# samxuxiang/BrepGen

Measured on NVIDIA H100. Metric: B-reps/sec (1000-step ABC cascade), higher is better.
Workload: dtype f16 x f16 -> f32 (wgmma; split hi+lo weights on in/out-proj; fp32 residual/LN/softmax)

## Files before the change

### brepgen_b200/_ffi.py

```python
from __future__ import annotations

import ctypes as C
import os
from typing import Optional

_HERE = os.path.dirname(os.path.abspath(__file__))
LIB_PATH = os.environ.get("BG_LIB", os.path.join(_HERE, "libbrepgen_b200.so"))

vp, i32, i64, u64, f32, sz = C.c_void_p, C.c_int, C.c_int64, C.c_uint64, C.c_float, C.c_size_t


class BgNamedTensor(C.Structure):
    _fields_ = [("name", C.c_char_p), ("data", vp), ("numel", i64)]


class BgDenoiserArgs(C.Structure):
    _fields_ = [("B", i32), ("S", i32), ("E", i32), ("x", vp), ("timesteps", vp), ("n_timesteps", i32),
                ("surfPos", vp), ("surfZ", vp), ("edgePos", vp), ("mask", vp), ("class_label", vp), ("out", vp), ("compact", i32)]


SIGNATURES = {
    "bg_version": (i32, []),
    "bg_last_error": (C.c_char_p, []),
    "bg_check_device": (i32, []),
    "bg_launch_count": (u64, []),
    "bg_denoiser_create": (i32, [i32, i32, i32, C.POINTER(BgNamedTensor), i32, vp, vp, C.POINTER(vp)]),
    "bg_denoiser_destroy": (None, [vp]),
    "bg_denoiser_workspace_bytes": (sz, [vp, i32, i32, i32]),
    "bg_denoiser_forward": (i32, [vp, C.POINTER(BgDenoiserArgs), vp, sz, vp]),
    "bg_vae_create": (i32, [i32, C.POINTER(BgNamedTensor), i32, vp, C.POINTER(vp)]),
    "bg_vae_destroy": (None, [vp]),
    "bg_vae_workspace_bytes": (sz, [vp, i32]),
    "bg_vae_decode": (i32, [vp, vp, i32, vp, vp, sz, vp]),
    "bg_vae_decode_hw": (i32, [vp, vp, i32, i32, vp, vp, sz, vp]),
    "bg_vae_encode": (i32, [vp, vp, i32, i32, vp, vp, sz, vp]),
    "bg_ddpm_step": (i32, [vp, vp, f32, vp, vp, vp, u64, u64, i64, f32, f32, f32, f32, f32, f32, vp]),
    "bg_ddpm_step_tab": (i32, [vp, vp, f32, vp, vp, u64, u64, u64, i64, vp, vp, f32, vp]),
    "bg_step_advance": (i32, [vp, i32, vp, vp, vp]),
    "bg_pndm_step": (i32, [vp, vp, i64, f32, f32, vp, f32, vp, f32, vp, f32, vp, f32, vp]),
    "bg_axpby": (i32, [vp, f32, vp, f32, vp, i64, vp]),
    "bg_dedup_surfaces": (i32, [vp, i32, i32, f32, vp, vp, vp]),
    "bg_dedup_edges": (i32, [vp, vp, i32, i32, i32, f32, vp, vp]),
    "bg_edge_endpoints": (i32, [vp, vp, f32, i64, vp, vp]),
    "bg_nn_exclude": (i32, [vp, vp, vp, i32, vp, vp]),
    "bg_pairs_within": (i32, [vp, i32, f32, vp, vp]),
    "bg_edge_pair_match": (i32, [vp, vp, i32, i32, f32, vp, vp]),
    "bg_edge_fit": (i32, [vp, vp, i32, vp, vp]),
    "bg_surf_init": (i32, [vp, vp, vp, vp, vp, i32, vp, vp]),
    "bg_surf_offset_opt": (i32, [vp, vp, vp, vp, vp, i32, i32, i32, f32, f32, f32, f32, f32, vp, vp, vp]),
    "bg_op_gemm_f16": (i32, [vp, i32, vp, i32, i32, i32, i32, vp, i32, i32, i32, vp, vp, i32, vp, i32, i32, vp]),
    "bg_op_attention": (i32, [vp, vp, i32, i32, vp, i32, vp, vp]),
    "bg_op_layernorm_f16": (i32, [vp, i32, vp, vp, vp, i32, i32, i32, vp]),
    "bg_op_cast_f16": (i32, [vp, vp, i64, vp]),
}

_lib: Optional[C.CDLL] = None


def lib() -> C.CDLL:
    global _lib
    if _lib is None:
        if not os.path.exists(LIB_PATH):
            raise RuntimeError(f"{LIB_PATH} not found: build it with `python -c 'import __graft_entry__ as g; g.build()'` "
                               "(brepgen_b200 has no CPU / PyTorch fallback)")
        l = C.CDLL(LIB_PATH)
        for name, (res, args) in SIGNATURES.items():
            fn = getattr(l, name)
            fn.restype, fn.argtypes = res, args
        _lib = l
    return _lib


def check(status: int, what: str = "") -> None:
    if status != 0:
        msg = lib().bg_last_error().decode(errors="replace")
        raise RuntimeError(f"brepgen_b200 {what} failed (status {status}): {msg}")


def ptr(t) -> Optional[int]:
    return None if t is None else t.data_ptr()


def named_tensors(state_dict, device):
    import torch
    arr = (BgNamedTensor * len(state_dict))()
    for i, (k, v) in enumerate(state_dict.items()):
        if v.device != device or v.dtype != torch.float32 or not v.is_contiguous():
            raise RuntimeError(f"parameter {k} must be contiguous fp32 on {device} (call .to(device) first)")
        arr[i].name, arr[i].data, arr[i].numel = k.encode(), v.data_ptr(), v.numel()
    return arr


def current_stream() -> int:
    import torch
    return torch.cuda.current_stream().cuda_stream


replayed_launches = 0


def note_replay(launches_per_replay: int, times: int = 1) -> None:
    global replayed_launches
    replayed_launches += int(launches_per_replay) * int(times)
```

### brepgen_b200/csrc/api.cu

```cuda
#include "../../include/brepgen_b200.h"
#include "bg_internal.h"

namespace bg {
const char* last_error_cstr();
}
using namespace bg;

extern "C" {

int bg_version(void) { return 100; }

const char* bg_last_error(void) { return last_error_cstr(); }

uint64_t bg_launch_count(void) { return launch_count(); }

int bg_check_device(void) {
  int dev = 0, major = 0, minor = 0;
  BG_CUDA(cudaGetDevice(&dev));
  BG_CUDA(cudaDeviceGetAttribute(&major, cudaDevAttrComputeCapabilityMajor, dev));
  BG_CUDA(cudaDeviceGetAttribute(&minor, cudaDevAttrComputeCapabilityMinor, dev));
  if (major != 9 || minor != 0)
    return set_error(BG_ERR_UNSUPPORTED_ARCH, "brepgen_b200 kernels are built for sm_90a (H100) only; device is sm_" +
                                                  std::to_string(major) + std::to_string(minor));
  return BG_OK;
}

int bg_op_gemm_f16(const void* A, int lda, const void* W, int ldw, int M, int N, int K, void* out, int ldo, int out_f16,
                   int relu, const float* bias, const float* resid, int ldr, const float* rowvec, int rows_per_vec,
                   int ldv, void* stream) {
  BG_TRY(bg_check_device());
  GemmEpilogue ep;
  ep.out = out; ep.ldo = ldo; ep.out_f16 = out_f16; ep.relu = relu; ep.bias = bias;
  ep.resid = resid; ep.ldr = ldr; ep.rowvec = rowvec; ep.rows_per_vec = rows_per_vec; ep.ldv = ldv;
  return launch_gemm_f16(reinterpret_cast<cudaStream_t>(stream), reinterpret_cast<const __half*>(A), lda,
                         reinterpret_cast<const __half*>(W), ldw, M, N, K, ep);
}

int bg_op_attention(const void* qkv, void* out, int B, int L, const uint8_t* key_mask, int use_block_list,
                    int* scratch_int, void* stream) {
  BG_TRY(bg_check_device());
  cudaStream_t st = reinterpret_cast<cudaStream_t>(stream);
  AttnArgs a;
  a.qkv = reinterpret_cast<const __half*>(qkv);
  a.out = reinterpret_cast<__half*>(out);
  a.ldo = 768; a.B = B; a.L = L; a.key_mask = key_mask;
  if (use_block_list && key_mask) {
    BG_REQUIRE(scratch_int != nullptr, "attention: block list needs scratch_int");
    const int nkb = (L + 127) / 128;
    a.blk_list = scratch_int;
    a.blk_count = scratch_int + (size_t)B * nkb;
    uint32_t* words = reinterpret_cast<uint32_t*>(scratch_int + (size_t)B * (nkb + 1));
    a.blk_words = words;
    BG_TRY(launch_build_block_list(st, key_mask, B, L, scratch_int, scratch_int + (size_t)B * nkb, words));
  }
  return launch_attention(st, a);
}

int bg_op_layernorm_f16(const float* x, int ldx, const float* gamma, const float* beta, void* y, int ldy, int rows,
                        int act, void* stream) {
  return launch_layernorm_f16(reinterpret_cast<cudaStream_t>(stream), x, ldx, gamma, beta, reinterpret_cast<__half*>(y),
                              ldy, rows, act);
}

int bg_op_cast_f16(const float* x, void* y, int64_t n, void* stream) {
  return launch_cast_f32_to_f16(reinterpret_cast<cudaStream_t>(stream), x, reinterpret_cast<__half*>(y), (size_t)n);
}

}
```

### brepgen_b200/csrc/attn.cu

```cuda
#include <math.h>

#include "bg_internal.h"
#include "ptx.cuh"


namespace bg {

namespace {

constexpr int DH = 64;
constexpr int NHEAD = 12;
constexpr int DMODEL = 768;
constexpr int BQ = 128;
constexpr int TILE_BYTES = 128 * DH * 2;
constexpr int ST = 2;
constexpr int OFF_Q = 0;
constexpr int OFF_K = TILE_BYTES;
constexpr int OFF_V = OFF_K + ST * TILE_BYTES;
constexpr int OFF_BAR = OFF_V + ST * TILE_BYTES;
constexpr int OFF_MASKW = OFF_BAR + 256;
constexpr int MAX_KB = 64;
constexpr int SMEM_BYTES = OFF_MASKW + MAX_KB * 16 + 1024;
constexpr int THREADS = 384;
constexpr int CONSUMER_THREADS = 256;

struct AttnParams {
  __half* out;
  int ldo;
  int B, L, nkb;
  const uint8_t* key_mask;
  const int* blk_list;
  const int* blk_count;
  const uint32_t* blk_words;
  const int* seq_row0;
  const int* seq_len;
  float scale_log2;
};

__device__ __forceinline__ float quad_max(float v) {
  v = fmaxf(v, __shfl_xor_sync(0xffffffffu, v, 1));
  return fmaxf(v, __shfl_xor_sync(0xffffffffu, v, 2));
}
__device__ __forceinline__ float quad_sum(float v) {
  v += __shfl_xor_sync(0xffffffffu, v, 1);
  return v + __shfl_xor_sync(0xffffffffu, v, 2);
}

__global__ void __launch_bounds__(THREADS, 1)
attn_kernel(const __grid_constant__ CUtensorMap tmQKV, const AttnParams p) {
  extern __shared__ uint8_t smem_raw[];
  uint8_t* smem = reinterpret_cast<uint8_t*>((reinterpret_cast<uintptr_t>(smem_raw) + 1023) & ~uintptr_t(1023));
  uint64_t* bars = reinterpret_cast<uint64_t*>(smem + OFF_BAR);
  uint64_t* q_full = bars;
  uint64_t* k_full = q_full + 1;
  uint64_t* k_empty = k_full + ST;
  uint64_t* v_full = k_empty + ST;
  uint64_t* v_empty = v_full + ST;

  const int warp = threadIdx.x >> 5;
  const int lane = threadIdx.x & 31;
  const int wg = threadIdx.x >> 7;
  const int qgrp = blockIdx.x, h = blockIdx.y, b = blockIdx.z;
  const int row0 = p.seq_row0 ? p.seq_row0[b] : b * p.L;
  const int len = p.seq_len ? p.seq_len[b] : p.L;
  if (qgrp * BQ >= len) return;
  const int nblk = p.blk_count ? p.blk_count[b] : (len + 127) / 128;
  const int* blist = p.blk_list ? p.blk_list + (size_t)b * p.nkb : nullptr;

  if (threadIdx.x == 0) {
    tma_prefetch_desc(&tmQKV);
    mbar_init(q_full, 1);
    for (int i = 0; i < ST; ++i) {
      mbar_init(&k_full[i], 1);
      mbar_init(&k_empty[i], CONSUMER_THREADS);
      mbar_init(&v_full[i], 1);
      mbar_init(&v_empty[i], CONSUMER_THREADS);
    }
    fence_barrier_init();
  }
  uint32_t* maskw = reinterpret_cast<uint32_t*>(smem + OFF_MASKW);
  if (p.blk_words || !p.key_mask) {
    for (int wi = threadIdx.x; wi < nblk * 4; wi += THREADS) {
      uint32_t w;
      if (p.blk_words) {
        w = p.blk_words[((size_t)b * p.nkb + (wi >> 2)) * 4 + (wi & 3)];
      } else {
        const int base = (wi >> 2) * 128 + (wi & 3) * 32;
        w = base + 32 <= len ? 0u : (base >= len ? 0xffffffffu : (0xffffffffu << (len - base)));
      }
      maskw[wi] = w;
    }
  } else {
    for (int wi = warp; wi < nblk * 4; wi += THREADS / 32) {
      const int kb = blist ? blist[wi >> 2] : (wi >> 2);
      const int key = kb * 128 + (wi & 3) * 32 + lane;
      bool bad = key >= len;
      if (!bad) bad = p.key_mask[(size_t)b * p.L + key] != 0;
      const uint32_t w = __ballot_sync(0xffffffffu, bad);
      if (lane == 0) maskw[wi] = w;
    }
  }
  __syncthreads();

  if (wg == 0) {
    setmaxnreg_dec<24>();
    if (warp == 0 && elect_one()) {
      mbar_arrive_expect_tx(q_full, TILE_BYTES);
      tma_load_2d(smem + OFF_Q, &tmQKV, q_full, h * DH, row0 + qgrp * BQ);
      for (int it = 0; it < nblk; ++it) {
        const int kb = blist ? blist[it] : it;
        const int s = it % ST;
        const uint32_t par = ((it / ST) & 1) ^ 1;
        mbar_wait(&k_empty[s], par);
        mbar_arrive_expect_tx(&k_full[s], TILE_BYTES);
        tma_load_2d(smem + OFF_K + s * TILE_BYTES, &tmQKV, &k_full[s], DMODEL + h * DH, row0 + kb * 128);
        mbar_wait(&v_empty[s], par);
        mbar_arrive_expect_tx(&v_full[s], TILE_BYTES);
        tma_load_2d(smem + OFF_V + s * TILE_BYTES, &tmQKV, &v_full[s], 2 * DMODEL + h * DH, row0 + kb * 128);
      }
    }
    return;
  }

  setmaxnreg_inc<240>();
  const int half = wg - 1;
  const int wq = warp & 3;
  const float c = p.scale_log2;
  const uint32_t q_addr = smem_u32(smem + OFF_Q) + half * 64 * 128;
  float m_run[2] = {-INFINITY, -INFINITY}, l_run[2] = {0.f, 0.f};
  float o[DH / 2];
#pragma unroll
  for (int i = 0; i < DH / 2; ++i) o[i] = 0.f;

  mbar_wait(q_full, 0);
  for (int it = 0; it < nblk; ++it) {
    const int s = it % ST;
    const uint32_t par = (it / ST) & 1;
    float sc[64];
    mbar_wait(&k_full[s], par);
    const uint32_t k_addr = smem_u32(smem + OFF_K + s * TILE_BYTES);
    wgmma_fence();
#pragma unroll
    for (int k = 0; k < DH / 16; ++k)
      wgmma_m64n128k16_ss(sc, make_sw128_desc(q_addr + k * 32), make_sw128_desc(k_addr + k * 32), k > 0 ? 1u : 0u);
    wgmma_commit();
    wgmma_wait<0>();
    wgmma_fence_operand(sc);
    mbar_arrive(&k_empty[s]);

    const uint4 iw = *reinterpret_cast<const uint4*>(maskw + it * 4);
    if ((iw.x | iw.y | iw.z | iw.w) != 0) {
      const uint32_t inval[4] = {iw.x, iw.y, iw.z, iw.w};
#pragma unroll
      for (int i = 0; i < 16; ++i)
#pragma unroll
        for (int j = 0; j < 2; ++j) {
          const int key = 8 * i + 2 * (lane & 3) + j;
          if ((inval[key >> 5] >> (key & 31)) & 1u) {
            sc[4 * i + j] = -INFINITY;
            sc[4 * i + 2 + j] = -INFINITY;
          }
        }
    }
    float ref[2], alpha[2];
#pragma unroll
    for (int hr = 0; hr < 2; ++hr) {
      float mx = -INFINITY;
#pragma unroll
      for (int i = 0; i < 16; ++i) mx = fmaxf(mx, fmaxf(sc[4 * i + 2 * hr], sc[4 * i + 2 * hr + 1]));
      const float m_new = fmaxf(m_run[hr], quad_max(mx));
      ref[hr] = m_new == -INFINITY ? 0.f : m_new;
      alpha[hr] = ex2((m_run[hr] - ref[hr]) * c);
      m_run[hr] = m_new;
      l_run[hr] *= alpha[hr];
    }
#pragma unroll
    for (int i = 0; i < DH / 8; ++i) {
      o[4 * i] *= alpha[0];
      o[4 * i + 1] *= alpha[0];
      o[4 * i + 2] *= alpha[1];
      o[4 * i + 3] *= alpha[1];
    }
    uint32_t pa[8][4];
    const float nm0 = -ref[0] * c, nm1 = -ref[1] * c;
#pragma unroll
    for (int i = 0; i < 16; ++i) {
      const float p0 = ex2(fmaf(sc[4 * i], c, nm0)), p1 = ex2(fmaf(sc[4 * i + 1], c, nm0));
      const float p2 = ex2(fmaf(sc[4 * i + 2], c, nm1)), p3 = ex2(fmaf(sc[4 * i + 3], c, nm1));
      l_run[0] += p0 + p1;
      l_run[1] += p2 + p3;
      pa[i >> 1][(i & 1) * 2] = pack_half2(p0, p1);
      pa[i >> 1][(i & 1) * 2 + 1] = pack_half2(p2, p3);
    }

    mbar_wait(&v_full[s], par);
    const uint32_t v_addr = smem_u32(smem + OFF_V + s * TILE_BYTES);
    wgmma_fence_operand(o);
    wgmma_fence();
#pragma unroll
    for (int kk = 0; kk < 8; ++kk) wgmma_m64n64k16_rs_bt(o, pa[kk], make_sw128_desc(v_addr + kk * 2048), 1u);
    wgmma_commit();
    wgmma_wait<0>();
    wgmma_fence_operand(o);
    mbar_arrive(&v_empty[s]);
  }

#pragma unroll
  for (int hr = 0; hr < 2; ++hr) {
    const float l = quad_sum(l_run[hr]);
    const float inv = l > 0.f ? 1.f / l : 0.f;
    const int row = qgrp * BQ + half * 64 + wq * 16 + hr * 8 + (lane >> 2);
    if (row >= len) continue;
    __half* dst = p.out + ((size_t)row0 + row) * p.ldo + h * DH + 2 * (lane & 3);
#pragma unroll
    for (int i = 0; i < DH / 8; ++i)
      *reinterpret_cast<uint32_t*>(dst + 8 * i) = pack_half2(o[4 * i + 2 * hr] * inv, o[4 * i + 2 * hr + 1] * inv);
  }
}

__global__ void block_list_kernel(const uint8_t* __restrict__ key_mask, int L, int nkb, int* __restrict__ blk_list,
                                  int* __restrict__ blk_count, uint32_t* __restrict__ blk_words) {
  extern __shared__ int sm_bl[];
  int* pos = sm_bl;
  uint32_t* wds = reinterpret_cast<uint32_t*>(sm_bl + nkb);
  const int b = blockIdx.x;
  const int warp = threadIdx.x >> 5, lane = threadIdx.x & 31, nwarp = blockDim.x >> 5;
  for (int kb = warp; kb < nkb; kb += nwarp) {
    bool any = false;
#pragma unroll
    for (int c = 0; c < 4; ++c) {
      const int key = kb * 128 + c * 32 + lane;
      const bool bad = key >= L || key_mask[(size_t)b * L + key] != 0;
      const uint32_t w = __ballot_sync(0xffffffffu, bad);
      any = any || w != 0xffffffffu;
      if (lane == 0) wds[kb * 4 + c] = w;
    }
    if (lane == 0) pos[kb] = any ? 0 : -1;
  }
  __syncthreads();
  if (threadIdx.x == 0) {
    int n = 0;
    for (int kb = 0; kb < nkb; ++kb)
      if (pos[kb] == 0) {
        blk_list[(size_t)b * nkb + n] = kb;
        pos[kb] = n++;
      }
    blk_count[b] = n;
  }
  __syncthreads();
  if (blk_words)
    for (int i = threadIdx.x; i < nkb * 4; i += blockDim.x)
      if (pos[i >> 2] >= 0) blk_words[((size_t)b * nkb + pos[i >> 2]) * 4 + (i & 3)] = wds[i];
}

}

int launch_attention(cudaStream_t st, const AttnArgs& a) {
  BG_REQUIRE(a.qkv && a.out && a.B > 0 && a.L > 0, "attention: bad arguments");
  BG_REQUIRE(a.ldo % 8 == 0, "attention: output pitch must be a multiple of 8");
  BG_REQUIRE(a.L <= 128 * MAX_KB, "attention: sequence longer than 8192 tokens is not supported");
  BG_REQUIRE((a.blk_list == nullptr) == (a.blk_count == nullptr), "attention: blk_list and blk_count go together");
  CUtensorMap tm;
  BG_REQUIRE((a.seq_row0 == nullptr) == (a.seq_len == nullptr), "attention: seq_row0 and seq_len go together");
  BG_REQUIRE(a.seq_len == nullptr || (a.key_mask == nullptr && a.blk_list == nullptr), "attention: variable-length mode takes no mask");
  BG_TRY(make_tmap_2d_f16(&tm, a.qkv, (uint64_t)a.B * (uint64_t)a.L, 3 * DMODEL, 3 * DMODEL, 128));
  AttnParams p;
  p.out = a.out; p.ldo = a.ldo; p.B = a.B; p.L = a.L; p.nkb = (a.L + 127) / 128;
  p.key_mask = a.key_mask; p.blk_list = a.blk_list; p.blk_count = a.blk_count; p.blk_words = a.blk_words;
  p.seq_row0 = a.seq_row0; p.seq_len = a.seq_len;
  p.scale_log2 = 1.4426950408889634f / 8.0f;
  BG_TRY(ensure_dynamic_smem(reinterpret_cast<const void*>(&attn_kernel), SMEM_BYTES));
  dim3 grid((a.L + BQ - 1) / BQ, NHEAD, a.B);
  attn_kernel<<<grid, THREADS, SMEM_BYTES, st>>>(tm, p);
  return check_launch("attn_kernel launch");
}

int launch_build_block_list(cudaStream_t st, const uint8_t* key_mask, int B, int L, int* blk_list, int* blk_count,
                            uint32_t* blk_words) {
  BG_REQUIRE(key_mask && blk_list && blk_count && B > 0 && L > 0, "block list: bad arguments");
  const int nkb = (L + 127) / 128;
  block_list_kernel<<<B, 128, nkb * 5 * sizeof(int), st>>>(key_mask, L, nkb, blk_list, blk_count, blk_words);
  return check_launch("block_list_kernel launch");
}

}
```

### include/brepgen_b200.h

```cpp
#ifndef BREPGEN_B200_H_
#define BREPGEN_B200_H_

#include <stddef.h>
#include <stdint.h>

#ifdef __cplusplus
extern "C" {
#endif

typedef enum {
  BG_STATUS_OK = 0,
  BG_STATUS_BAD_ARG = -1,
  BG_STATUS_UNSUPPORTED_ARCH = -2,
  BG_STATUS_CUDA = -3,
  BG_STATUS_WORKSPACE = -4,
  BG_STATUS_MISSING_WEIGHT = -5
} BgStatus;

int bg_version(void);
const char* bg_last_error(void);
uint64_t bg_launch_count(void);
int bg_check_device(void);

typedef struct BgDenoiser BgDenoiser;

typedef struct {
  const char* name;
  const float* data;
  int64_t numel;
} BgNamedTensor;

int bg_denoiser_create(int kind, int use_cf, int precision, const BgNamedTensor* weights, int n_weights,
                       const float* sincos, void* stream, BgDenoiser** out);
void bg_denoiser_destroy(BgDenoiser* m);

typedef struct {
  int B, S, E;
  const float* x;
  const int64_t* timesteps;
  int n_timesteps;
  const float* surfPos;
  const float* surfZ;
  const float* edgePos;
  const uint8_t* mask;
  const int64_t* class_label;
  float* out;
  int compact;
} BgDenoiserArgs;

size_t bg_denoiser_workspace_bytes(const BgDenoiser* m, int B, int S, int E);
int bg_denoiser_forward(BgDenoiser* m, const BgDenoiserArgs* args, void* workspace, size_t workspace_bytes,
                        void* stream);

typedef struct BgVae BgVae;
int bg_vae_create(int kind, const BgNamedTensor* weights, int n_weights, void* stream, BgVae** out);
void bg_vae_destroy(BgVae* m);
size_t bg_vae_workspace_bytes(const BgVae* m, int N);
int bg_vae_decode(BgVae* m, const float* z, int N, float* out, void* workspace, size_t workspace_bytes, void* stream);
int bg_vae_decode_hw(BgVae* m, const float* z, int N, int hw, float* out, void* workspace, size_t workspace_bytes,
                     void* stream);
int bg_vae_encode(BgVae* m, const float* x, int N, int hw, float* out, void* workspace, size_t workspace_bytes,
                  void* stream);

int bg_ddpm_step(const float* eps_cond, const float* eps_uncond, float cfg_w, const float* x, float* out,
                 const float* noise, uint64_t seed, uint64_t offset, int64_t n, float sqrt_one_minus_abar,
                 float sqrt_abar, float clip, float c_x0, float c_x, float sigma, void* stream);
int bg_ddpm_step_tab(const float* eps_cond, const float* eps_uncond, float cfg_w, const float* x, float* out, uint64_t seed,
                     uint64_t offset0, uint64_t offset_stride, int64_t n, const float* coef_table, const int32_t* step,
                     float clip, void* stream);
int bg_step_advance(const int64_t* timesteps, int n_steps, int32_t* step, int64_t* t_cur, void* stream);
int bg_pndm_step(const float* x, float* out, int64_t n, float c_sample, float c_eps, const float* e0, float w0,
                 const float* e1, float w1, const float* e2, float w2, const float* e3, float w3, void* stream);
int bg_axpby(const float* x, float a, const float* y, float b, float* out, int64_t n, void* stream);

int bg_dedup_surfaces(const float* surfPos, int B, int S, float threshold, float* out_pos, uint8_t* out_mask, void* stream);
int bg_dedup_edges(const float* edgePos, const uint8_t* surf_mask, int B, int S, int E, float threshold,
                   uint8_t* edge_mask, void* stream);

int bg_op_gemm_f16(const void* A, int lda, const void* W, int ldw, int M, int N, int K, void* out, int ldo, int out_f16,
                   int relu, const float* bias, const float* resid, int ldr, const float* rowvec, int rows_per_vec,
                   int ldv, void* stream);
int bg_op_attention(const void* qkv, void* out, int B, int L, const uint8_t* key_mask, int use_block_list,
                    int* scratch_int, void* stream);
int bg_op_layernorm_f16(const float* x, int ldx, const float* gamma, const float* beta, void* y, int ldy, int rows,
                        int act, void* stream);
int bg_op_cast_f16(const float* x, void* y, int64_t n, void* stream);

int bg_edge_endpoints(const float* edge_ncs, const float* edge_pos, float pos_scale, int64_t n_edges, float* out, void* stream);
int bg_nn_exclude(const float* pts, const int32_t* group, const int32_t* seg_off, int n_seg, int32_t* nn, void* stream);
int bg_pairs_within(const float* pts, int n, float threshold, uint8_t* out, void* stream);
int bg_edge_pair_match(const int32_t* edge_vertex_adj, const float* z, int z_dim, int n, float threshold, uint8_t* out,
                       void* stream);
int bg_edge_fit(const float* edge_ncs, const float* vertex_se, int n_edges, float* edge_wcs, void* stream);
int bg_surf_init(const float* surf_ncs, const float* surf_pos, const float* edge_wcs, const int32_t* adj_off, const int32_t* adj,
                 int n_faces, float* surf_wcs, void* stream);
int bg_surf_offset_opt(const float* surf_init, const float* edge_wcs, const int32_t* adj_off, const int32_t* adj,
                       const float* inv_nface, int n_faces, int max_edges_per_face, int iters, float lr, float beta1, float beta2,
                       float eps, float weight_decay, float* surf_out, float* offset_out, void* stream);

#ifdef __cplusplus
}
#endif
#endif
```

Measured before the change: 0.1608.

## Software-pipeline attention QK and PV wgmma across key blocks; add varlen entry

Restructures the attention consumer loop so the QK^T wgmma for block it is issued together with the PV wgmma for block it-1, letting softmax of one block overlap tensor-core work of the next. Stage and phase bookkeeping moves into a small ring struct, and the softmax, rescale and pack steps are factored into helpers. It also adds a variable-length attention API that passes per-sequence row offsets and lengths. This adds register pressure (sc, pa and o are live together) and more complex barrier ordering for the V buffers. The varlen path relies on AttnArgs fields and kernel support that are not visible here.

```diff
diff --git a/brepgen_b200/_ffi.py b/brepgen_b200/_ffi.py
--- a/brepgen_b200/_ffi.py
+++ b/brepgen_b200/_ffi.py
@@ -50,6 +50,7 @@
     "bg_surf_offset_opt": (i32, [vp, vp, vp, vp, vp, i32, i32, i32, f32, f32, f32, f32, f32, vp, vp, vp]),
     "bg_op_gemm_f16": (i32, [vp, i32, vp, i32, i32, i32, i32, vp, i32, i32, i32, vp, vp, i32, vp, i32, i32, vp]),
     "bg_op_attention": (i32, [vp, vp, i32, i32, vp, i32, vp, vp]),
+    "bg_op_attention_varlen": (i32, [vp, vp, i32, i32, vp, vp, vp]),
     "bg_op_layernorm_f16": (i32, [vp, i32, vp, vp, vp, i32, i32, i32, vp]),
     "bg_op_cast_f16": (i32, [vp, vp, i64, vp]),
 }
diff --git a/brepgen_b200/csrc/api.cu b/brepgen_b200/csrc/api.cu
--- a/brepgen_b200/csrc/api.cu
+++ b/brepgen_b200/csrc/api.cu
@@ -56,6 +56,18 @@
   return launch_attention(st, a);
 }
 
+int bg_op_attention_varlen(const void* qkv, void* out, int B, int L, const int* seq_row0, const int* seq_len,
+                           void* stream) {
+  BG_TRY(bg_check_device());
+  BG_REQUIRE(seq_row0 && seq_len, "attention: variable-length mode needs seq_row0 and seq_len");
+  AttnArgs a;
+  a.qkv = reinterpret_cast<const __half*>(qkv);
+  a.out = reinterpret_cast<__half*>(out);
+  a.ldo = 768; a.B = B; a.L = L;
+  a.seq_row0 = seq_row0; a.seq_len = seq_len;
+  return launch_attention(reinterpret_cast<cudaStream_t>(stream), a);
+}
+
 int bg_op_layernorm_f16(const float* x, int ldx, const float* gamma, const float* beta, void* y, int ldy, int rows,
                         int act, void* stream) {
   return launch_layernorm_f16(reinterpret_cast<cudaStream_t>(stream), x, ldx, gamma, beta, reinterpret_cast<__half*>(y),
diff --git a/brepgen_b200/csrc/attn.cu b/brepgen_b200/csrc/attn.cu
--- a/brepgen_b200/csrc/attn.cu
+++ b/brepgen_b200/csrc/attn.cu
@@ -46,6 +46,90 @@
   return v + __shfl_xor_sync(0xffffffffu, v, 2);
 }
 
+struct Ring {
+  int stage = 0;
+  uint32_t phase = 0;
+  __device__ __forceinline__ void advance() {
+    if (++stage == ST) {
+      stage = 0;
+      phase ^= 1u;
+    }
+  }
+};
+
+__device__ __forceinline__ void issue_qk(float (&sc)[64], uint32_t q_addr, uint32_t k_addr) {
+#pragma unroll
+  for (int k = 0; k < DH / 16; ++k)
+    wgmma_m64n128k16_ss(sc, make_sw128_desc(q_addr + k * 32), make_sw128_desc(k_addr + k * 32), k > 0 ? 1u : 0u);
+  wgmma_commit();
+}
+
+__device__ __forceinline__ void issue_pv(float (&o)[DH / 2], const uint32_t (&pa)[8][4], uint32_t v_addr) {
+#pragma unroll
+  for (int kk = 0; kk < 8; ++kk) wgmma_m64n64k16_rs_bt(o, pa[kk], make_sw128_desc(v_addr + kk * 2048), 1u);
+  wgmma_commit();
+}
+
+__device__ __forceinline__ void softmax_block(float (&sc)[64], const uint32_t* iw4, float (&m_run)[2], float (&l_run)[2],
+                                              float (&alpha)[2], float c, int lane) {
+  const uint4 iw = *reinterpret_cast<const uint4*>(iw4);
+  if ((iw.x | iw.y | iw.z | iw.w) != 0) {
+    const uint32_t inval[4] = {iw.x, iw.y, iw.z, iw.w};
+#pragma unroll
+    for (int i = 0; i < 16; ++i)
+#pragma unroll
+      for (int j = 0; j < 2; ++j) {
+        const int key = 8 * i + 2 * (lane & 3) + j;
+        if ((inval[key >> 5] >> (key & 31)) & 1u) {
+          sc[4 * i + j] = -INFINITY;
+          sc[4 * i + 2 + j] = -INFINITY;
+        }
+      }
+  }
+  float ref[2];
+#pragma unroll
+  for (int hr = 0; hr < 2; ++hr) {
+    float mx = -INFINITY;
+#pragma unroll
+    for (int i = 0; i < 16; ++i) mx = fmaxf(mx, fmaxf(sc[4 * i + 2 * hr], sc[4 * i + 2 * hr + 1]));
+    const float m_new = fmaxf(m_run[hr], quad_max(mx));
+    ref[hr] = m_new == -INFINITY ? 0.f : m_new;
+    alpha[hr] = ex2((m_run[hr] - ref[hr]) * c);
+    m_run[hr] = m_new;
+    l_run[hr] *= alpha[hr];
+  }
+  const float nm0 = -ref[0] * c, nm1 = -ref[1] * c;
+#pragma unroll
+  for (int i = 0; i < 16; ++i) {
+    const float p0 = ex2(fmaf(sc[4 * i], c, nm0)), p1 = ex2(fmaf(sc[4 * i + 1], c, nm0));
+    const float p2 = ex2(fmaf(sc[4 * i + 2], c, nm1)), p3 = ex2(fmaf(sc[4 * i + 3], c, nm1));
+    l_run[0] += p0 + p1;
+    l_run[1] += p2 + p3;
+    sc[4 * i] = p0;
+    sc[4 * i + 1] = p1;
+    sc[4 * i + 2] = p2;
+    sc[4 * i + 3] = p3;
+  }
+}
+
+__device__ __forceinline__ void scale_o(float (&o)[DH / 2], const float (&alpha)[2]) {
+#pragma unroll
+  for (int i = 0; i < DH / 8; ++i) {
+    o[4 * i] *= alpha[0];
+    o[4 * i + 1] *= alpha[0];
+    o[4 * i + 2] *= alpha[1];
+    o[4 * i + 3] *= alpha[1];
+  }
+}
+
+__device__ __forceinline__ void pack_p(uint32_t (&pa)[8][4], const float (&sc)[64]) {
+#pragma unroll
+  for (int i = 0; i < 16; ++i) {
+    pa[i >> 1][(i & 1) * 2] = pack_half2(sc[4 * i], sc[4 * i + 1]);
+    pa[i >> 1][(i & 1) * 2 + 1] = pack_half2(sc[4 * i + 2], sc[4 * i + 3]);
+  }
+}
+
 __global__ void __launch_bounds__(THREADS, 1)
 attn_kernel(const __grid_constant__ CUtensorMap tmQKV, const AttnParams p) {
   extern __shared__ uint8_t smem_raw[];
@@ -107,14 +191,14 @@
     if (warp == 0 && elect_one()) {
       mbar_arrive_expect_tx(q_full, TILE_BYTES);
       tma_load_2d(smem + OFF_Q, &tmQKV, q_full, h * DH, row0 + qgrp * BQ);
-      for (int it = 0; it < nblk; ++it) {
+      Ring r;
+      for (int it = 0; it < nblk; ++it, r.advance()) {
         const int kb = blist ? blist[it] : it;
-        const int s = it % ST;
-        const uint32_t par = ((it / ST) & 1) ^ 1;
-        mbar_wait(&k_empty[s], par);
+        const int s = r.stage;
+        mbar_wait(&k_empty[s], r.phase ^ 1u);
         mbar_arrive_expect_tx(&k_full[s], TILE_BYTES);
         tma_load_2d(smem + OFF_K + s * TILE_BYTES, &tmQKV, &k_full[s], DMODEL + h * DH, row0 + kb * 128);
-        mbar_wait(&v_empty[s], par);
+        mbar_wait(&v_empty[s], r.phase ^ 1u);
         mbar_arrive_expect_tx(&v_full[s], TILE_BYTES);
         tma_load_2d(smem + OFF_V + s * TILE_BYTES, &tmQKV, &v_full[s], 2 * DMODEL + h * DH, row0 + kb * 128);
       }
@@ -133,76 +217,59 @@
   for (int i = 0; i < DH / 2; ++i) o[i] = 0.f;
 
   mbar_wait(q_full, 0);
-  for (int it = 0; it < nblk; ++it) {
-    const int s = it % ST;
-    const uint32_t par = (it / ST) & 1;
-    float sc[64];
-    mbar_wait(&k_full[s], par);
-    const uint32_t k_addr = smem_u32(smem + OFF_K + s * TILE_BYTES);
+  if (nblk > 0) {
+    const uint32_t k_base = smem_u32(smem + OFF_K), v_base = smem_u32(smem + OFF_V);
+    Ring kr, vr;
+    float sc[64], alpha[2];
+    uint32_t pa[8][4];
+
+    mbar_wait(&k_full[kr.stage], kr.phase);
     wgmma_fence();
-#pragma unroll
-    for (int k = 0; k < DH / 16; ++k)
-      wgmma_m64n128k16_ss(sc, make_sw128_desc(q_addr + k * 32), make_sw128_desc(k_addr + k * 32), k > 0 ? 1u : 0u);
-    wgmma_commit();
+    issue_qk(sc, q_addr, k_base + kr.stage * TILE_BYTES);
     wgmma_wait<0>();
     wgmma_fence_operand(sc);
-    mbar_arrive(&k_empty[s]);
-
-    const uint4 iw = *reinterpret_cast<const uint4*>(maskw + it * 4);
-    if ((iw.x | iw.y | iw.z | iw.w) != 0) {
-      const uint32_t inval[4] = {iw.x, iw.y, iw.z, iw.w};
-#pragma unroll
-      for (int i = 0; i < 16; ++i)
-#pragma unroll
-        for (int j = 0; j < 2; ++j) {
-          const int key = 8 * i + 2 * (lane & 3) + j;
-          if ((inval[key >> 5] >> (key & 31)) & 1u) {
-            sc[4 * i + j] = -INFINITY;
-            sc[4 * i + 2 + j] = -INFINITY;
-          }
-        }
-    }
-    float ref[2], alpha[2];
-#pragma unroll
-    for (int hr = 0; hr < 2; ++hr) {
-      float mx = -INFINITY;
-#pragma unroll
-      for (int i = 0; i < 16; ++i) mx = fmaxf(mx, fmaxf(sc[4 * i + 2 * hr], sc[4 * i + 2 * hr + 1]));
-      const float m_new = fmaxf(m_run[hr], quad_max(mx));
-      ref[hr] = m_new == -INFINITY ? 0.f : m_new;
-      alpha[hr] = ex2((m_run[hr] - ref[hr]) * c);
-      m_run[hr] = m_new;
-      l_run[hr] *= alpha[hr];
-    }
-#pragma unroll
-    for (int i = 0; i < DH / 8; ++i) {
-      o[4 * i] *= alpha[0];
-      o[4 * i + 1] *= alpha[0];
-      o[4 * i + 2] *= alpha[1];
-      o[4 * i + 3] *= alpha[1];
-    }
-    uint32_t pa[8][4];
-    const float nm0 = -ref[0] * c, nm1 = -ref[1] * c;
-#pragma unroll
-    for (int i = 0; i < 16; ++i) {
-      const float p0 = ex2(fmaf(sc[4 * i], c, nm0)), p1 = ex2(fmaf(sc[4 * i + 1], c, nm0));
-      const float p2 = ex2(fmaf(sc[4 * i + 2], c, nm1)), p3 = ex2(fmaf(sc[4 * i + 3], c, nm1));
-      l_run[0] += p0 + p1;
-      l_run[1] += p2 + p3;
-      pa[i >> 1][(i & 1) * 2] = pack_half2(p0, p1);
-      pa[i >> 1][(i & 1) * 2 + 1] = pack_half2(p2, p3);
-    }
-
-    mbar_wait(&v_full[s], par);
-    const uint32_t v_addr = smem_u32(smem + OFF_V + s * TILE_BYTES);
+    mbar_arrive(&k_empty[kr.stage]);
+    kr.advance();
+    softmax_block(sc, maskw, m_run, l_run, alpha, c, lane);
+
+#pragma unroll 1
+    for (int it = 1; it < nblk; ++it) {
+      wgmma_wait<0>();
+      wgmma_fence_operand(o);
+      if (it >= 2) {
+        mbar_arrive(&v_empty[vr.stage]);
+        vr.advance();
+      }
+      scale_o(o, alpha);
+      pack_p(pa, sc);
+      mbar_wait(&k_full[kr.stage], kr.phase);
+      mbar_wait(&v_full[vr.stage], vr.phase);
+      wgmma_fence_operand(o);
+      wgmma_fence();
+      issue_qk(sc, q_addr, k_base + kr.stage * TILE_BYTES);
+      issue_pv(o, pa, v_base + vr.stage * TILE_BYTES);
+      wgmma_wait<1>();
+      wgmma_fence_operand(sc);
+      mbar_arrive(&k_empty[kr.stage]);
+      kr.advance();
+      softmax_block(sc, maskw + it * 4, m_run, l_run, alpha, c, lane);
+    }
+
+    wgmma_wait<0>();
+    wgmma_fence_operand(o);
+    if (nblk >= 2) {
+      mbar_arrive(&v_empty[vr.stage]);
+      vr.advance();
+    }
+    scale_o(o, alpha);
+    pack_p(pa, sc);
+    mbar_wait(&v_full[vr.stage], vr.phase);
     wgmma_fence_operand(o);
     wgmma_fence();
-#pragma unroll
-    for (int kk = 0; kk < 8; ++kk) wgmma_m64n64k16_rs_bt(o, pa[kk], make_sw128_desc(v_addr + kk * 2048), 1u);
-    wgmma_commit();
+    issue_pv(o, pa, v_base + vr.stage * TILE_BYTES);
     wgmma_wait<0>();
     wgmma_fence_operand(o);
-    mbar_arrive(&v_empty[s]);
+    mbar_arrive(&v_empty[vr.stage]);
   }
 
 #pragma unroll
diff --git a/include/brepgen_b200.h b/include/brepgen_b200.h
--- a/include/brepgen_b200.h
+++ b/include/brepgen_b200.h
@@ -82,6 +82,8 @@
                    int ldv, void* stream);
 int bg_op_attention(const void* qkv, void* out, int B, int L, const uint8_t* key_mask, int use_block_list,
                     int* scratch_int, void* stream);
+int bg_op_attention_varlen(const void* qkv, void* out, int B, int L, const int* seq_row0, const int* seq_len,
+                           void* stream);
 int bg_op_layernorm_f16(const float* x, int ldx, const float* gamma, const float* beta, void* y, int ldy, int rows,
                         int act, void* stream);
 int bg_op_cast_f16(const float* x, void* y, int64_t n, void* stream);
```

New measurement: 0.1689 (median of 6 runs). 5.0% higher.
